# huggingface/open-muse

Hardware: AMD Instinct MI355X
Metric: images/sec/node (MaskGit train step, 256^2, bs=64/GPU) (higher is better)
Workload: dtype bf16 (transformer GEMM/attention operands; f32 accumulate, residual, norms, loss) + bf16x3 tokenizer (f32 activations, f32-class products as 3 bf16 MFMAs); parity of this mode was not measured in this run (a --full run measures it); 1 GPU; MaskGit train step: MaskGitVQGAN f16-256 encode (bf16x3) + cosine mask + MaskGitTransformer config B (configs/imagenet.yaml: hidden 768, 24 layers, 16 heads, vocab 2048, seq 257) fwd+bwd (bf16 MFMA, f32 accum/residual) + AdamW; global_batch=64, per_gpu_batch=64, resolution=256, seq_len=257, parallelism=dp1, vqgan_dtype=bf16x3, random_init=True, wgrad_stream=True

## Files before the change

include/muse_hip.h:

```cpp
#ifndef MUSE_HIP_H
#define MUSE_HIP_H
#include <stdint.h>

#ifdef __cplusplus
extern "C" {
#endif

enum { MUSE_F32 = 0, MUSE_BF16 = 1, MUSE_F16 = 2  };
enum { MUSE_ERR_BAD_ARG = -1, MUSE_ERR_ALIGN = -2, MUSE_ERR_UNSUPPORTED = -3 };

int muse_version(void);

typedef struct muse_gemm_desc {
  const void* A;
  const void* B;
  void* C;
  const void* bias;
  const void* rowvec;
  const void* residual;
  int32_t dtype;
  int32_t out_dtype;
  int32_t layout_a, layout_b;
  int32_t M, N, K;
  int32_t batch, zdiv;
  int64_t lda, ldb, ldc, ldr;
  int64_t sA0, sA1, sB0, sB1, sC0, sC1;
  float alpha;
  int32_t accumulate;
  int32_t act;
  int32_t split_k;
  int64_t split_stride;
} muse_gemm_desc;
int muse_gemm(const muse_gemm_desc* d, void* stream);
int muse_gemm_tile(const muse_gemm_desc* d);
int muse_gemm_x3(const muse_gemm_desc* d, int64_t a_lo, int64_t b_lo, void* stream);
int muse_gemm_path(const muse_gemm_desc* d);

int muse_gemm_group_ok(const muse_gemm_desc* d, int32_t n, int32_t split_k);
int muse_gemm_group(const muse_gemm_desc* d, int32_t n, int32_t split_k, void* stream);

int muse_transpose(const void* in, void* out, int32_t dtype, int32_t rows, int32_t cols, int64_t ld_in, int64_t ld_out,
                   int32_t batch, int64_t stride_in, int64_t stride_out, void* stream);

int muse_layernorm_fwd(const void* x, int32_t x_dtype, const float* w, const float* residual, void* y, int32_t y_dtype,
                       float* mean, float* rstd, int32_t rows, int32_t cols, float eps, void* stream);
int muse_layernorm_bwd(const void* dy, int32_t dy_dtype, const void* x, int32_t x_dtype, const float* w,
                       const float* mean, const float* rstd, const float* dres, void* dx, int32_t dx_dtype,
                       void* dx_bf16, float* dw_partial, int32_t nblk, int32_t rows, int32_t cols, void* stream);
int muse_layernorm_bwd_nblk(int32_t rows);
int muse_layernorm_pair_fwd(const void* ao, const float* x, const float* w_post, const float* w_pre, float* x1, void* ln2,
                            float* mean_post, float* rstd_post, float* mean_pre, float* rstd_pre, int32_t rows, int32_t cols,
                            float eps, void* stream);
int muse_layernorm_pair_bwd(const void* dln2, const float* x1, const float* w_pre, const float* mean_pre, const float* rstd_pre,
                            const float* dres, const void* ao, const float* w_post, const float* mean_post, const float* rstd_post,
                            float* dx1, void* dao, float* dw_partial_pre, float* dw_partial_post, int32_t nblk, int32_t rows,
                            int32_t cols, void* stream);
int muse_colsum(const float* in, float* out, int32_t rows, int32_t cols, int32_t accumulate, void* stream);
int muse_add_rowvec(float* x, const float* b, int64_t rows, int32_t cols, void* stream);
int muse_bias_grad_rows_per_block(void);
int muse_bias_grad_partial(const void* dy, int32_t dtype, float* partial, int64_t rows, int32_t cols, int64_t ld, void* stream);

int muse_softmax_fwd(const void* x, void* y, int32_t dtype, int64_t rows, int32_t cols, int64_t ld, void* stream);
int muse_softmax_bwd(const void* p, const void* dp, void* ds, int32_t dtype, int64_t rows, int32_t cols, int64_t ld,
                     void* stream);

typedef struct muse_attn_desc {
  const void* q;
  const void* k;
  const void* v;
  void* o;
  int64_t ldq, ldk, ldv, ldo;
  int64_t bsq, bsk, bsv, bso;
  int32_t batch, heads, head_dim, seq_q, seq_kv;
  float alpha;
} muse_attn_desc;
int muse_attention_seq_pad(int32_t seq);
int muse_attention_fwd_ex(const muse_attn_desc* d, float* lse, void* stream);
int muse_attention_bwd_ex(const muse_attn_desc* d, const void* d_o, int64_t lddo, int64_t bsdo, const float* lse, float* dsum,
                          void* dq, int64_t lddq, int64_t bsdq, void* dk, int64_t lddk, int64_t bsdk, void* dv, int64_t lddv,
                          int64_t bsdv, void* stream);
int muse_attention_x3_fwd(const muse_attn_desc* d, float* lse, void* o_planes, int64_t o_lo, int32_t half, float scale, int32_t* stats,
                          void* stream);
int muse_attention_x3_bwd(const muse_attn_desc* d, const void* d_o, int64_t lddo, int64_t bsdo, const float* lse, void* dq,
                          int64_t lddq, int64_t bsdq, void* dk, int64_t lddk, int64_t bsdk, void* dv, int64_t lddv, int64_t bsdv,
                          void* dq_planes, int64_t dq_lo, void* dk_planes, int64_t dk_lo, void* dv_planes, int64_t dv_lo, int32_t half,
                          float scale, int32_t* stats, void* stream);
int muse_attention_x3_fwd_stream(const muse_attn_desc* d, float* lse, void* o_planes, int64_t o_lo, int32_t half, float scale,
                                 int32_t* stats, void* stream);
int muse_attention_x3_bwd_stream(const muse_attn_desc* d, const float* d_o, int64_t lddo, int64_t bsdo, const float* lse, float* dsum,
// ... 211 lines not shown
```

open-muse_amd/csrc/gemm.hip:

```cpp
#include "gemm_core.h"
#include "gemm256.h"
#include "gemm_p.h"
#include "../../include/muse_hip.h"

template <typename T, typename TC, int BM>
static int dispatch_bm(const GemmParams& p, int la, int lb, int batch, hipStream_t s) {
  constexpr int NT = BM * 2;
  if (la == 0 && lb == 0) return launch_gemm<T, TC, 0, 0, BM, PlainLoader<T, 0, BM, NT>, PlainLoader<T, 0, 128, NT>>(p, batch, s);
  if (la == 0 && lb == 1) return launch_gemm<T, TC, 0, 1, BM, PlainLoader<T, 0, BM, NT>, PlainLoader<T, 1, 128, NT>>(p, batch, s);
  if (la == 1 && lb == 1) return launch_gemm<T, TC, 1, 1, BM, PlainLoader<T, 1, BM, NT>, PlainLoader<T, 1, 128, NT>>(p, batch, s);
  if (la == 1 && lb == 0) return launch_gemm<T, TC, 1, 0, BM, PlainLoader<T, 1, BM, NT>, PlainLoader<T, 0, 128, NT>>(p, batch, s);
  return MUSE_ERR_BAD_ARG;
}
template <typename T, typename TC>
static int dispatch_layout(const GemmParams& p, int la, int lb, int batch, hipStream_t s) {
  return use_bm256(p, batch) ? dispatch_bm<T, TC, 256>(p, la, lb, batch, s) : dispatch_bm<T, TC, 128>(p, la, lb, batch, s);
}

static int fill_params(const muse_gemm_desc* d, GemmParams& p) {
  if (!d || !d->A || !d->B || !d->C) return MUSE_ERR_BAD_ARG;
  const int esz = (d->dtype == MUSE_BF16 || d->dtype == MUSE_F16) ? 2 : 4;
  const int ch = 16 / esz;
  if ((d->lda % ch) || (d->ldb % ch) || (((uintptr_t)d->A) & 15) || (((uintptr_t)d->B) & 15)) return MUSE_ERR_ALIGN;
  if ((d->sA0 % ch) || (d->sA1 % ch) || (d->sB0 % ch) || (d->sB1 % ch)) return MUSE_ERR_ALIGN;
  {
    const int64_t ra = d->layout_a == 0 ? d->M : d->K, ca = d->layout_a == 0 ? d->K : d->M;
    const int64_t rb = d->layout_b == 0 ? d->N : d->K, cb = d->layout_b == 0 ? d->K : d->N;
    if (((ra - 1) * d->lda + ca + ch) * esz >= (1LL << 32) || ((rb - 1) * d->ldb + cb + ch) * esz >= (1LL << 32)) return MUSE_ERR_UNSUPPORTED;
  }
  p.A = d->A; p.B = d->B; p.C = d->C;
  p.bias = (const float*)d->bias; p.rowvec = (const float*)d->rowvec; p.residual = d->residual;
  p.M = d->M; p.N = d->N; p.K = d->K;
  p.lda = d->lda; p.ldb = d->ldb; p.ldc = d->ldc; p.ldr = d->ldr;
  p.zdiv = d->zdiv > 0 ? d->zdiv : 1;
  p.sA0 = d->sA0; p.sA1 = d->sA1; p.sB0 = d->sB0; p.sB1 = d->sB1; p.sC0 = d->sC0; p.sC1 = d->sC1;
  p.alpha = d->alpha; p.accumulate = d->accumulate; p.act = d->act;
  p.split_k = d->split_k > 1 ? d->split_k : 1;
  p.split_stride = p.split_k > 1 ? d->split_stride : 0;
  if (p.split_k > 1 && (d->out_dtype != MUSE_F32 || d->bias || d->rowvec || d->residual || d->act)) return MUSE_ERR_BAD_ARG;
  p.cH = p.cW = p.cCin = p.cKS = p.cUps = 0; p.cCinShift = -1;
  p.a_lo = p.b_lo = 0;
  return 0;
}

static bool takes_gemm256(const muse_gemm_desc* d, const GemmParams& p, int batch) {
  if (d->dtype == MUSE_F16) {
    return d->out_dtype == MUSE_F32 && d->M >= 128 && d->N >= 128 && d->K >= 64 && gemm256_ok<float>(p, d->layout_a, d->layout_b);
  }
  if (d->dtype != MUSE_BF16) return false;
  const bool pers = (d->out_dtype == MUSE_BF16 || d->out_dtype == MUSE_F32) &&
                    gemm256p_takes(p, d->layout_a, d->layout_b, batch, d->out_dtype == MUSE_F32);
  if (!gemm256_preferred(p, d->layout_a, d->layout_b, batch, pers)) return false;
  if (d->out_dtype == MUSE_BF16) return gemm256_ok<bf16_t>(p, d->layout_a, d->layout_b);
  if (d->out_dtype == MUSE_F32) return gemm256_ok<float>(p, d->layout_a, d->layout_b);
  return false;
}

extern "C" int muse_gemm_tile(const muse_gemm_desc* d) {
  GemmParams p;
  const int rc = fill_params(d, p);
  if (rc) return rc;
  if (takes_gemm256(d, p, d->batch > 0 ? d->batch : 1)) return 256;
  return d->dtype == MUSE_F16 ? MUSE_ERR_UNSUPPORTED : 128;
}

extern "C" int muse_gemm_path(const muse_gemm_desc* d) {
  GemmParams p;
  const int rc = fill_params(d, p);
  if (rc) return rc;
  const int batch = d->batch > 0 ? d->batch : 1;
  if (!takes_gemm256(d, p, batch)) return d->dtype == MUSE_F16 ? MUSE_ERR_UNSUPPORTED : 128;
  return gemm256p_takes(p, d->layout_a, d->layout_b, batch, d->out_dtype == MUSE_F32) ? 257 : 256;
}

extern "C" int muse_gemm(const muse_gemm_desc* d, void* stream) {
  GemmParams p;
  const int rc = fill_params(d, p);
  if (rc) return rc;
  const int batch = d->batch > 0 ? d->batch : 1;
  hipStream_t s = (hipStream_t)stream;
  if (d->dtype == MUSE_F16 && !takes_gemm256(d, p, batch)) return MUSE_ERR_UNSUPPORTED;
  if (takes_gemm256(d, p, batch)) {
    const bool half_ops = d->dtype == MUSE_F16;
    if (gemm256p_takes(p, d->layout_a, d->layout_b, batch, d->out_dtype == MUSE_F32)) {
      const int rp = launch_gemm256p(p, d->layout_a, d->layout_b, d->out_dtype == MUSE_F32, s, half_ops);
      if (rp != -1) return rp;
    }
    if (half_ops) return launch_gemm256_f16(p, d->layout_a, d->layout_b, batch, s);
    if (d->out_dtype == MUSE_BF16) return launch_gemm256<bf16_t>(p, d->layout_a, d->layout_b, batch, s);
    return launch_gemm256<float>(p, d->layout_a, d->layout_b, batch, s);
  }
  if (d->dtype == MUSE_BF16) {
    if (d->out_dtype == MUSE_BF16) return dispatch_layout<bf16_t, bf16_t>(p, d->layout_a, d->layout_b, batch, s);
    if (d->out_dtype == MUSE_F32) return dispatch_layout<bf16_t, float>(p, d->layout_a, d->layout_b, batch, s);
  } else if (d->dtype == MUSE_F32 && d->out_dtype == MUSE_F32) {
    return dispatch_layout<float, float>(p, d->layout_a, d->layout_b, batch, s);
  }
  return MUSE_ERR_BAD_ARG;
}

extern "C" int muse_gemm_x3(const muse_gemm_desc* d, int64_t a_lo, int64_t b_lo, void* stream) {
  GemmParams p;
  const int rc = fill_params(d, p);
  if (rc) return rc;
  if (d->dtype != MUSE_BF16 || d->out_dtype != MUSE_F32 || d->batch > 1 || d->act) return MUSE_ERR_UNSUPPORTED;
  if (a_lo <= 0 || b_lo <= 0 || (a_lo & 7) || (b_lo & 7)) return MUSE_ERR_ALIGN;
  if (d->M < 128 || d->N < 128 || d->K < 64 || !gemm256_ok<float>(p, d->layout_a, d->layout_b)) return MUSE_ERR_UNSUPPORTED;
  {
    p.a_lo = a_lo; p.b_lo = b_lo;
  }
  return launch_gemm256_x3<float>(p, d->layout_a, d->layout_b, (hipStream_t)stream);
}

static int group_fill(const muse_gemm_desc* d, int n, int split_k, g256::GroupParams& gp) {
  if (!d || n < 1 || n > g256::MAXG || split_k < 1) return MUSE_ERR_BAD_ARG;
  int start = 0;
  for (int i = 0; i < n; ++i) {
    if ((d[i].dtype != MUSE_BF16 && d[i].dtype != MUSE_F16) || d[i].dtype != d[0].dtype || d[i].out_dtype != MUSE_F32 || d[i].layout_a != 1 ||
        d[i].layout_b != 1)
      return MUSE_ERR_UNSUPPORTED;
    if ((d[i].batch > 1) || d[i].bias || d[i].rowvec || d[i].residual || d[i].act) return MUSE_ERR_UNSUPPORTED;
    muse_gemm_desc di = d[i];
    di.split_k = split_k;
    if (split_k > 1 && di.split_stride == 0) return MUSE_ERR_BAD_ARG;
    const int rc = fill_params(&di, gp.p[i]);
// ... 30 lines not shown
```

open-muse_amd/csrc/gemm256p.h:

```cpp
#pragma once
#include "gemm256.h"

namespace g256p {
using namespace g256;

constexpr int TK_OFF = LDS_BYTES;
constexpr int LDS_BYTES_P = LDS_BYTES + 64;

struct Sched {
  int ntm_full, ntn, nstrip, q, r;
  __host__ __device__ int count(int x) const {
    const int s0 = (x - r) & 7;
    return q + (x < r ? 1 : 0) + (s0 < nstrip ? (nstrip - s0 + 7) / 8 : 0);
  }
  __device__ __forceinline__ bool decode(int x, int l, int& m0, int& n0) const {
    const int full = q + (x < r ? 1 : 0);
    if (l < 0) return false;
    if (l < full) {
      const int id = (x < r ? x * (q + 1) : r * (q + 1) + (x - r) * q) + l;
      constexpr int GM = 4;
      const int grp = id / (GM * ntn), first_m = grp * GM;
      const int gm = min(ntm_full - first_m, GM), in_grp = id - grp * (GM * ntn);
      m0 = (first_m + in_grp % gm) * BM;
      n0 = (in_grp / gm) * BN;
      return true;
    }
    const int s = ((x - r) & 7) + 8 * (l - full);
    if (s < nstrip) { m0 = ntm_full * BM; n0 = s * BN; return true; }
    return false;
  }
};

struct PArgs {
  GemmParams g;
  Sched sched;
  unsigned* counters;
  int nk2;
  int dyn;
  int epi;
  int staux;
  int stagger;
};

template <int L>
struct DmaP {
  rsrc_t rs;
  unsigned voff0[4];
  unsigned kk0, oob, kstep, ld2;
  unsigned vmask;
  unsigned r0off;
  int kend, R, rel0;
  __device__ __forceinline__ void init(const bf16_t* ptr, long ld, int R_, int K, int wave, int lane) {
    kend = K; R = R_;
    const long cols = L == 0 ? K : R_, rows = L == 0 ? R_ : K;
    const unsigned bytes = (unsigned)(((rows - 1) * ld + (cols + 7) / 8 * 8) * 2);
    rs = make_rsrc(ptr, bytes);
    oob = (bytes + 15u) & ~15u;
    ld2 = (unsigned)(ld * 2);
    vmask = 0; r0off = 0;
    if constexpr (L == 0) {
      const int r8 = lane >> 3, pc = lane & 7;
      kstep = 128u;
      kk0 = (unsigned)((pc ^ (r8 >> 1)) * 8);
      rel0 = wave * 32 + r8;
#pragma unroll
      for (int j = 0; j < 4; ++j) {
        const int row = (wave * 4 + j) * 8 + r8;
        const int csrc = pc ^ ((row >> 1) & 7);
        voff0[j] = (unsigned)(((long)row * ld + csrc * 8) * 2);
      }
    } else {
      const int half = lane >> 5, pos = lane & 31;
      kstep = (unsigned)(64 * ld * 2);
      kk0 = (unsigned)(wave * 8 + half);
      rel0 = 0;
#pragma unroll
      for (int j = 0; j < 4; ++j) {
        const int kr = wave * 8 + j * 2 + half;
        const int csrc = pos ^ (km_sw(kr) << 1);
        voff0[j] = (unsigned)(((long)kr * ld + csrc * 8) * 2);
      }
    }
  }
  __device__ __forceinline__ int rel(int j, int wave, int lane) const {
    if constexpr (L == 0) return rel0 + 8 * j;
    const int half = lane >> 5, pos = lane & 31, kr = wave * 8 + j * 2 + half;
    return (pos ^ (km_sw(kr) << 1)) * 8;
  }
  __device__ __forceinline__ void set_tile(int r0, bool valid, int wave, int lane) {
    unsigned m = 0;
#pragma unroll
    for (int j = 0; j < 4; ++j) m |= (valid && (r0 + rel(j, wave, lane)) < R) ? (1u << j) : 0u;
    vmask = m;
    r0off = L == 0 ? (unsigned)r0 * ld2 : (unsigned)r0 * 2u;
  }
  __device__ __forceinline__ unsigned kk(int j) const { return L == 0 ? (kk0 ^ ((unsigned)(j & 1) << 5)) : (kk0 + 2u * j); }
  template <int LDS_OFF, int J>
  __device__ __forceinline__ void issue1(unsigned char* smem, int kt, int wave) const {
    const bool ok = ((unsigned)kt * 64u + kk(J)) < (unsigned)kend && ((vmask >> J) & 1u);
    const unsigned vo = ok ? voff0[J] : oob;
    __builtin_amdgcn_raw_ptr_buffer_load_lds(rs, (lds_void_t*)(smem + LDS_OFF + (wave * 4 + J) * 1024), 16, (int)vo,
                                             (int)((unsigned)kt * kstep + r0off), 0, 0);
  }
  template <int LDS_OFF>
  __device__ __forceinline__ void issue(unsigned char* smem, int kt, int wave) const {
    issue1<LDS_OFF, 0>(smem, kt, wave); issue1<LDS_OFF, 1>(smem, kt, wave);
    issue1<LDS_OFF, 2>(smem, kt, wave); issue1<LDS_OFF, 3>(smem, kt, wave);
  }
};

enum { M_NORMAL = 0, M_FIRST = 1, M_LAST = 2, M_PUBLISH = 3 };

template <typename TC, int AL, int BL, bool H = false>
struct PipeP {
  static constexpr bool F32OUT = sizeof(TC) == 4;
  static constexpr int RA = AL ? 2 : 1, RB = BL ? 2 : 1, NB = NI * RB;
  static constexpr int NSLOT = 4, DIST = NSLOT - 1;
  static constexpr int GB1 = 8 - DIST, GBAR = 16 - DIST;
  static constexpr int NST = F32OUT ? 32 : 16;
  DmaP<AL> da;
  DmaP<BL> db;
  Frags<AL, MI> fa;
  Frags<BL, NI> fb;
  f32x4 acc[MI][NI];
  bf16x8 ring[NSLOT];
  bf16x8 bk[2][NI];
  unsigned char* smem;
  Sched sched;
  unsigned* counters;
  int nk2, dyn, epi, staux, stagger, M, N;
  unsigned ldc;
  float alpha;
// ... 136 lines not shown
  }

  __device__ __forceinline__ void epilogue(int m0, int n0) {
    if (alpha != 1.f) {
#pragma unroll
      for (int i = 0; i < MI; ++i)
#pragma unroll
        for (int j = 0; j < NI; ++j) acc[i][j] *= alpha;
    }
    if (epi == 3) {
#pragma unroll
      for (int i = 0; i < MI; ++i)
        asm volatile("" ::"v"(acc[i][0]), "v"(acc[i][1]), "v"(acc[i][2]), "v"(acc[i][3]));
      return;
    }
    int ln = lane;
    asm volatile("" : "+v"(ln));
    const int pr = ln & 15, g = ln >> 4;
    const int rowlim = M - m0 - wr - pr;
    constexpr unsigned E = (unsigned)sizeof(TC);
    const unsigned soff = (unsigned)m0 * ldc * E + (unsigned)n0 * E, rstep = 16u * ldc * E;
    const unsigned rowb = (unsigned)(wr + pr) * ldc * E;
    if constexpr (F32OUT) {
      const int cb = wc + 4 * g;
      unsigned vb[NI];
#pragma unroll
      for (int j = 0; j < NI; ++j) vb[j] = (n0 + cb + 16 * j) < N ? rowb + (unsigned)(cb + 16 * j) * 4u : oobC;
#pragma unroll
      for (int i = 0; i < MI; ++i) {
        const bool rowok = 16 * i < rowlim;
#pragma unroll
        for (int j = 0; j < NI; ++j)
          __builtin_amdgcn_raw_buffer_store_b128(__builtin_bit_cast(u32x4, acc[i][j]), rsC, (int)(rowok ? vb[j] : oobC),
                                                 (int)(soff + (unsigned)i * rstep), 0);
        __builtin_amdgcn_sched_barrier(0);
      }
    } else {
      if (epi == 0) {
        const int cb = wc + 4 * g;
        unsigned vb[NI];
#pragma unroll
        for (int j = 0; j < NI; ++j) vb[j] = (n0 + cb + 16 * j) < N ? rowb + (unsigned)(cb + 16 * j) * 2u : oobC;
#pragma unroll
        for (int i = 0; i < MI; ++i) {
          const bool rowok = 16 * i < rowlim;
#pragma unroll
          for (int j = 0; j < NI; ++j) {
            const u32x2 w = {pack2_bf16(acc[i][j][0], acc[i][j][1]), pack2_bf16(acc[i][j][2], acc[i][j][3])};
            __builtin_amdgcn_raw_buffer_store_b64(w, rsC, (int)(rowok ? vb[j] : oobC), (int)(soff + (unsigned)i * rstep), 0);
          }
          __builtin_amdgcn_sched_barrier(0);
        }
      } else {
        const int cg = 16 * (g & 1) + 8 * (g >> 1);
        if (epi == 1) {
          unsigned vb[2];
#pragma unroll
          for (int q = 0; q < 2; ++q) vb[q] = (n0 + wc + cg + 32 * q) < N ? rowb + (unsigned)(wc + cg + 32 * q) * 2u : oobC;
#pragma unroll
          for (int i = 0; i < MI; ++i) {
            const bool rowok = 16 * i < rowlim;
#pragma unroll
            for (int q = 0; q < 2; ++q) {
              u32x4 w;
              swapped_chunk(i, q, w);
              store16(w, rowok ? vb[q] : oobC, soff + (unsigned)i * rstep);
            }
            __builtin_amdgcn_sched_barrier(0);
          }
        } else {
          const int odd = pr & 1;
          const int col = wc + cg + 32 * odd;
          const int rl0 = rowlim + odd;
          const unsigned vb0 = (n0 + col) < N ? rowb - (unsigned)odd * ldc * 2u + (unsigned)col * 2u : oobC;
          const unsigned vb1 = (n0 + col) < N ? vb0 + ldc * 2u : oobC;
#pragma unroll
          for (int i = 0; i < MI; ++i) {
            u32x4 c0, c1, d0, d1;
            swapped_chunk(i, 0, c0);
            swapped_chunk(i, 1, c1);
#pragma unroll
            for (int e = 0; e < 4; ++e) {
              const unsigned from1 = (unsigned)__builtin_amdgcn_update_dpp(0, (int)c1[e], 0xB1, 0xf, 0xf, false);
              const unsigned from0 = (unsigned)__builtin_amdgcn_update_dpp(0, (int)c0[e], 0xB1, 0xf, 0xf, false);
              d0[e] = odd ? from1 : c0[e];
              d1[e] = odd ? c1[e] : from0;
            }
            store16(d0, 16 * i < rl0 ? vb0 : oobC, soff + (unsigned)i * rstep);
            store16(d1, 16 * i + 1 < rl0 ? vb1 : oobC, soff + (unsigned)i * rstep);
            __builtin_amdgcn_sched_barrier(0);
          }
        }
      }
    }
  }

  __device__ __forceinline__ void tiles(int& m0, int& n0) {
    for (;;) {
      ktile<0, M_FIRST>();
      ktile<1, M_PUBLISH>();
      for (int it = 2; it < nk2 - 2; it += 2) {
        ktile<0, M_NORMAL>();
        ktile<1, M_NORMAL>();
      }
      ktile<0, M_LAST>();
      ktile<1, M_NORMAL>();
      issue_piece<1, 3>(1); issue_piece<1, 4>(1); issue_piece<1, 5>(1); issue_piece<1, 6>(1); issue_piece<1, 7>(1);
      fence();
      epilogue(m0, n0);
      fence();
      if (!has_next) return;
      m0 = nm0; n0 = nn0;
      const bool ld = init_acc(m0, n0);
      fence();
      pend = !ld && epi != 3;
    }
  }

  __device__ __forceinline__ void run(int m0, int n0) {
    if (dyn && stagger > 1) {
      const long wait = (long)((blockIdx.x >> 3) % stagger) * ((long)nk2 * 2500L / stagger);
      const long t0 = (long)__builtin_amdgcn_s_memtime();
      while ((long)__builtin_amdgcn_s_memtime() - t0 < wait) __builtin_amdgcn_s_sleep(16);
    }
    da.set_tile(m0, true, wave, lane);
    db.set_tile(n0, true, wave, lane);
    da.template issue<A_BASE>(smem, 0, wave);
    db.template issue<B_BASE>(smem, 0, wave);
    da.template issue<A_BASE + TILE>(smem, 1, wave);
    db.template issue<B_BASE + TILE>(smem, 1, wave);
    fence();
    const bool loads = init_acc(m0, n0);
    fence();
    if (loads) asm volatile("s_waitcnt vmcnt(40)" ::: "memory");
    else asm volatile("s_waitcnt vmcnt(8)" ::: "memory");
    __builtin_amdgcn_s_barrier();
    __builtin_amdgcn_sched_barrier(0);
    fb.template read_range<0, 0, 0, NI>(bk[0]);
    prologue_a<0>();
    __builtin_amdgcn_sched_barrier(0);
    kti = 0;
    pend = false;
    has_next = false;
    tiles(m0, n0);
    asm volatile("s_waitcnt vmcnt(0) lgkmcnt(0)" ::: "memory");
  }
};

template <typename TC, int AL, int BL, bool H = false>
__global__ __launch_bounds__(512, 2) void kernel(PArgs a) {
  extern __shared__ __attribute__((aligned(16))) unsigned char smem[];
  const GemmParams& p = a.g;
  const int lane = threadIdx.x & 63, wave = __builtin_amdgcn_readfirstlane(threadIdx.x >> 6);
  const int xcd = blockIdx.x & 7, nbx = gridDim.x >> 3;

  int m0, n0;
  if (a.sched.decode(xcd, blockIdx.x >> 3, m0, n0)) {
    PipeP<TC, AL, BL, H> pp;
    pp.smem = smem; pp.sched = a.sched; pp.counters = a.counters; pp.nk2 = a.nk2; pp.dyn = a.dyn; pp.epi = a.epi; pp.staux = a.staux; pp.stagger = a.stagger;
    pp.M = p.M; pp.N = p.N; pp.ldc = (unsigned)p.ldc; pp.alpha = p.alpha;
    pp.wave = wave; pp.lane = lane; pp.xcd = xcd; pp.nbx = nbx;
    pp.wr = (wave >> 2) * 128; pp.wc = (wave & 3) * 64;
    pp.tk = 0;
    pp.da.init((const bf16_t*)p.A, p.lda, p.M, p.K, wave, lane);
    pp.db.init((const bf16_t*)p.B, p.ldb, p.N, p.K, wave, lane);
    pp.fa.init(A_BASE, pp.wr, lane);
    pp.fb.init(B_BASE, pp.wc, lane);
    {
      const unsigned bytes = (unsigned)(((long)(p.M - 1) * p.ldc + p.N) * (long)sizeof(TC));
      pp.rsC = make_rsrc(p.C, bytes);
      pp.oobC = (bytes + 15u) & ~15u;
    }
    pp.init_src = nullptr; pp.ldI = 0; pp.oobI = 0; pp.rsI = pp.rsC;
    if constexpr (sizeof(TC) == 4) {
      if (p.residual || p.accumulate) {
        pp.init_src = p.residual ? p.residual : (const void*)p.C;
        pp.ldI = (unsigned)(p.residual ? p.ldr : p.ldc);
        const unsigned bytes = (unsigned)(((long)(p.M - 1) * pp.ldI + p.N) * 4L);
        pp.rsI = make_rsrc(pp.init_src, bytes);
        pp.oobI = (bytes + 15u) & ~15u;
      }
    }
    pp.run(m0, n0);
  }
  if (a.dyn && threadIdx.x == 0) {
    const unsigned left = __hip_atomic_fetch_add(a.counters + 8, 1u, __ATOMIC_RELAXED, __HIP_MEMORY_SCOPE_AGENT);
    if (left == gridDim.x - 1) {
#pragma unroll
      for (int x = 0; x < 9; ++x) __hip_atomic_exchange(a.counters + x, 0u, __ATOMIC_RELAXED, __HIP_MEMORY_SCOPE_AGENT);
    }
  }
}

}
```

open-muse_amd/csrc/gemm_p.h:

```cpp
#pragma once
#include "gemm_core.h"
bool gemm256p_takes(const GemmParams& p, int la, int lb, int batch, bool f32_out);
int launch_gemm256p(const GemmParams& p, int la, int lb, bool f32_out, hipStream_t stream, bool half_ops = false);
```

open-muse_amd/csrc/gemm_p.hip:

```cpp
#include "gemm256p.h"
#include "gemm_p.h"
#include <mutex>
#include <stdio.h>

namespace {

constexpr int kMaxDev = 16;
struct Slots {
  unsigned* base = nullptr;
  hipStream_t streams[64];
  int n = 0;
  int cus = 0;
  bool failed = false;
};
std::mutex g_mu;
Slots g_slots[kMaxDev];

Slots* slots_of_current_device() {
  int dev = 0;
  if (hipGetDevice(&dev) != hipSuccess || dev < 0 || dev >= kMaxDev) { (void)hipGetLastError(); return nullptr; }
  Slots& S = g_slots[dev];
  if (S.failed) return nullptr;
  if (!S.base) {
    hipDeviceProp_t prop;
    if (hipGetDeviceProperties(&prop, dev) != hipSuccess || hipMalloc((void**)&S.base, 64 * 64) != hipSuccess ||
        hipMemset(S.base, 0, 64 * 64) != hipSuccess) {
      (void)hipGetLastError();
      S.failed = true;
      S.base = nullptr;
      return nullptr;
    }
    S.cus = prop.multiProcessorCount;
  }
  return &S;
}

unsigned* counters_for(hipStream_t s, int* cus) {
  std::lock_guard<std::mutex> lk(g_mu);
  hipStreamCaptureStatus cap = hipStreamCaptureStatusNone;
  if (hipStreamIsCapturing(s, &cap) != hipSuccess) (void)hipGetLastError();
  if (cap != hipStreamCaptureStatusNone) return nullptr;
  Slots* S = slots_of_current_device();
  if (!S) return nullptr;
  *cus = S->cus;
  for (int i = 0; i < S->n; ++i)
    if (S->streams[i] == s) return S->base + i * 16;
  if (S->n == 64) return nullptr;
  S->streams[S->n] = s;
  return S->base + (S->n++) * 16;
}

#define P_REJECT(why) do { if (getenv("MUSE_G256P_DEBUG")) fprintf(stderr, "[g256p] %dx%dx%d la%d lb%d out%d: %s\n", p.M, p.N, p.K, la, lb, (int)sizeof(TC), why); return false; } while (0)
template <typename TC>
bool eligible(const GemmParams& p, int la, int lb, int batch) {
  constexpr long E = (long)sizeof(TC);
  if (batch != 1 || p.split_k > 1 || p.act != 0 || p.bias || p.rowvec) P_REJECT("batch / split-K / activation / bias / row vector");
  if (la != 0 || (sizeof(TC) == 4 && lb != 0)) P_REJECT("operand layout");
  if (p.K <= 128) P_REJECT("K <= 128");
  if (sizeof(TC) == 2 && (p.residual || p.accumulate)) P_REJECT("bf16 residual / accumulate");
  if (sizeof(TC) == 4 && ((p.residual && p.accumulate) || ((p.residual || p.accumulate) && p.alpha != 1.f))) P_REJECT("residual + accumulate / alpha");
  if (!gemm256_ok<TC>(p, la, lb)) P_REJECT("gemm256_ok");
  const long ra = la == 0 ? p.M : p.K, rb = lb == 0 ? p.N : p.K;
  if ((ra * p.lda + 16) * 2 >= (1L << 31) || (rb * p.ldb + 16) * 2 >= (1L << 31)) P_REJECT("operand >= 2 GiB");
  if (((long)p.M * p.ldc + 16) * E >= (1L << 31)) P_REJECT("C >= 2 GiB");
  if (p.residual && ((long)p.M * p.ldr + 16) * E >= (1L << 31)) P_REJECT("residual >= 2 GiB");
  return true;
}

template <typename TC, int AL, int BL, bool H = false>
int launch(const GemmParams& p, hipStream_t stream) {
  int cus = 0;
  unsigned* counters = counters_for(stream, &cus);
  if (!counters || cus < 8) {
    if (getenv("MUSE_G256P_DEBUG")) fprintf(stderr, "[g256p] no queue slot (counters %p, %d CUs)\n", (void*)counters, cus);
    return -1;
  }
  g256p::PArgs a;
  a.g = p;
  a.counters = counters;
  g256p::Sched& sc = a.sched;
  sc.ntm_full = p.M / 256;
  sc.ntn = (p.N + 255) / 256;
  sc.nstrip = (p.M % 256) ? sc.ntn : 0;
  const int nfull = sc.ntm_full * sc.ntn;
  sc.q = nfull / 8; sc.r = nfull % 8;
  int longest = 0;
  for (int x = 0; x < 8; ++x) longest = sc.count(x) > longest ? sc.count(x) : longest;
  const int per_xcd = cus / 8;
  const int nbx = longest < per_xcd ? longest : per_xcd;
  a.dyn = longest > nbx;
  a.nk2 = (((p.K + 63) / 64) + 1) & ~1;
  static const int epi = []() { const char* e = getenv("MUSE_G256P_EPI"); return e ? atoi(e) : 2; }();
  a.epi = epi;
  static const int staux = []() { const char* e = getenv("MUSE_G256P_STAUX"); return e ? atoi(e) : 0; }();
  static const int stagger = []() { const char* e = getenv("MUSE_G256P_STAGGER"); return e ? atoi(e) : 1; }();
  a.staux = staux;
  a.stagger = stagger;
  auto kern = g256p::kernel<TC, AL, BL, H>;
  set_max_dynamic_lds((const void*)kern, g256p::LDS_BYTES_P);
  hipLaunchKernelGGL(kern, dim3(8 * nbx), dim3(512), g256p::LDS_BYTES_P, stream, a);
  return (int)hipGetLastError();
}

int launch_l(const GemmParams& p, int la, int lb, bool f32_out, hipStream_t s, bool half_ops) {
  if (la != 0) return -1;
  if (half_ops) return (f32_out && lb == 0) ? launch<float, 0, 0, true>(p, s) : -1;
  if (f32_out) return lb == 0 ? launch<float, 0, 0>(p, s) : -1;
  return lb == 0 ? launch<bf16_t, 0, 0>(p, s) : launch<bf16_t, 0, 1>(p, s);
}

}

bool gemm256p_takes(const GemmParams& p, int la, int lb, int batch, bool f32_out) {
  const char* e = getenv("MUSE_G256P");
  if (e && e[0] == '0') return false;
  return f32_out ? eligible<float>(p, la, lb, batch) : eligible<bf16_t>(p, la, lb, batch);
}

int launch_gemm256p(const GemmParams& p, int la, int lb, bool f32_out, hipStream_t stream, bool half_ops) {
  return launch_l(p, la, lb, f32_out, stream, half_ops);
}
```

open-muse_amd/muse/_hip.py:

```python
from __future__ import annotations

import ctypes as C
import os

import torch

F32, BF16, F16 = 0, 1, 2
_HERE = os.path.dirname(os.path.abspath(__file__))
LIB_PATH = os.environ.get("MUSE_HIP_LIB") or os.path.join(_HERE, "libmuse_hip.so")
_lib = None

c_void_p, c_int, c_i64, c_float = C.c_void_p, C.c_int32, C.c_int64, C.c_float


class GemmDesc(C.Structure):
    _fields_ = [
        ("A", c_void_p), ("B", c_void_p), ("C", c_void_p),
        ("bias", c_void_p), ("rowvec", c_void_p), ("residual", c_void_p),
        ("dtype", c_int), ("out_dtype", c_int), ("layout_a", c_int), ("layout_b", c_int),
        ("M", c_int), ("N", c_int), ("K", c_int), ("batch", c_int), ("zdiv", c_int),
        ("lda", c_i64), ("ldb", c_i64), ("ldc", c_i64), ("ldr", c_i64),
        ("sA0", c_i64), ("sA1", c_i64), ("sB0", c_i64), ("sB1", c_i64), ("sC0", c_i64), ("sC1", c_i64),
        ("alpha", c_float), ("accumulate", c_int), ("act", c_int), ("split_k", c_int), ("split_stride", c_i64),
    ]


class AttnDesc(C.Structure):
    _fields_ = [
        ("q", c_void_p), ("k", c_void_p), ("v", c_void_p), ("o", c_void_p),
        ("ldq", c_i64), ("ldk", c_i64), ("ldv", c_i64), ("ldo", c_i64),
        ("bsq", c_i64), ("bsk", c_i64), ("bsv", c_i64), ("bso", c_i64),
        ("batch", c_int), ("heads", c_int), ("head_dim", c_int), ("seq_q", c_int), ("seq_kv", c_int),
        ("alpha", c_float),
    ]


_IMG = (c_int, c_float, c_void_p)

SIGNATURES = {
    "muse_version": [],
    "muse_gemm": [C.POINTER(GemmDesc), c_void_p],
    "muse_gemm_x3": [C.POINTER(GemmDesc), c_i64, c_i64, c_void_p],
    "muse_gemm_tile": [C.POINTER(GemmDesc)],
    "muse_gemm_path": [C.POINTER(GemmDesc)],
    "muse_transpose": [c_void_p, c_void_p, c_int, c_int, c_int, c_i64, c_i64, c_int, c_i64, c_i64, c_void_p],
    "muse_layernorm_fwd": [c_void_p, c_int, c_void_p, c_void_p, c_void_p, c_int, c_void_p, c_void_p, c_int, c_int,
                           c_float, c_void_p],
    "muse_layernorm_bwd": [c_void_p, c_int, c_void_p, c_int, c_void_p, c_void_p, c_void_p, c_void_p, c_void_p, c_int,
                           c_void_p, c_void_p, c_int, c_int, c_int, c_void_p],
    "muse_layernorm_bwd_nblk": [c_int],
    "muse_layernorm_pair_fwd": [c_void_p] * 10 + [c_int, c_int, c_float, c_void_p],
    "muse_layernorm_pair_bwd": [c_void_p] * 14 + [c_int, c_int, c_int, c_void_p],
    "muse_colsum": [c_void_p, c_void_p, c_int, c_int, c_int, c_void_p],
    "muse_add_rowvec": [c_void_p, c_void_p, c_i64, c_int, c_void_p],
    "muse_bias_grad_rows_per_block": [],
    "muse_bias_grad_partial": [c_void_p, c_int, c_void_p, c_i64, c_int, c_i64, c_void_p],
    "muse_softmax_fwd": [c_void_p, c_void_p, c_int, c_i64, c_int, c_i64, c_void_p],
    "muse_softmax_bwd": [c_void_p, c_void_p, c_void_p, c_int, c_i64, c_int, c_i64, c_void_p],
    "muse_attention_seq_pad": [c_int],
    "muse_attention_fwd_ex": [C.POINTER(AttnDesc), c_void_p, c_void_p],
    "muse_attention_bwd_ex": [C.POINTER(AttnDesc), c_void_p, c_i64, c_i64, c_void_p, c_void_p, c_void_p, c_i64, c_i64, c_void_p,
                              c_i64, c_i64, c_void_p, c_i64, c_i64, c_void_p],
    "muse_attention_x3_fwd": [C.POINTER(AttnDesc), c_void_p, c_void_p, c_i64, *_IMG, c_void_p],
    "muse_attention_x3_bwd": [C.POINTER(AttnDesc), c_void_p, c_i64, c_i64, c_void_p, c_void_p, c_i64, c_i64, c_void_p, c_i64, c_i64, c_void_p,
                              c_i64, c_i64, c_void_p, c_i64, c_void_p, c_i64, c_void_p, c_i64, *_IMG, c_void_p],
    "muse_attention_x3_fwd_stream": [C.POINTER(AttnDesc), c_void_p, c_void_p, c_i64, *_IMG, c_void_p],
    "muse_attention_x3_bwd_stream": [C.POINTER(AttnDesc), c_void_p, c_i64, c_i64, c_void_p, c_void_p, c_void_p, c_i64, c_i64, c_void_p, c_i64, c_i64,
                                     c_void_p, c_i64, c_i64, c_void_p, c_i64, c_void_p, c_i64, c_void_p, c_i64, *_IMG, c_void_p],
    "muse_attention_x3_merge": [c_void_p, c_i64, c_void_p, c_i64, c_int, c_void_p, c_void_p, c_void_p, c_i64, c_int, c_int, c_int, *_IMG,
                                c_void_p],
    "muse_sum_parts_strided": [c_void_p, c_i64, c_int, c_i64, c_int, c_void_p, c_i64, c_int, c_void_p],
    "muse_attention_fwd": [c_void_p, c_void_p, c_void_p, c_int, c_int, c_int, c_int, c_float, c_void_p],
    "muse_attention_bwd": [c_void_p, c_void_p, c_void_p, c_void_p, c_void_p, c_void_p, c_int, c_int, c_int, c_int, c_float,
                           c_void_p],
    "muse_glu_fwd": [c_void_p, c_void_p, c_int, c_i64, c_int, c_void_p],
    "muse_glu_bwd": [c_void_p, c_void_p, c_void_p, c_int, c_i64, c_int, c_void_p],
    "muse_glu_fwd_x3": [c_void_p, c_void_p, c_void_p, c_i64, c_int, *_IMG, c_void_p],
    "muse_glu_bwd_x3": [c_void_p, c_void_p, c_void_p, c_void_p, c_i64, c_int, *_IMG, c_void_p],
    "muse_ffn_mid_rows_per_block": [],
    "muse_ffn_mid_fwd": [c_void_p, c_void_p, c_void_p, c_void_p, c_void_p, c_void_p, c_int, c_int, c_int, c_float, c_void_p],
    "muse_ffn_mid_bwd": [c_void_p, c_void_p, c_void_p, c_void_p, c_void_p, c_void_p, c_void_p, c_void_p, c_int, c_int, c_int,
                         c_void_p],
    "muse_gelu_fwd": [c_void_p, c_void_p, c_int, c_i64, c_void_p],
    "muse_gelu_bwd": [c_void_p, c_void_p, c_void_p, c_int, c_i64, c_void_p],
    "muse_gelu_bwd_f32_bf16": [c_void_p, c_void_p, c_void_p, c_i64, c_void_p],
    "muse_embed_fwd": [c_void_p, c_void_p, c_void_p, c_void_p, c_int, c_int, c_int, c_int, c_void_p],
    "muse_embed_bwd": [c_void_p, c_void_p, c_void_p, c_void_p, c_void_p, c_int, c_int, c_int, c_int, c_int, c_void_p],
    "muse_embed_bwd_scratch_floats": [c_int, c_int],
    "muse_embed_bwd2": [c_void_p, c_void_p, c_void_p, c_void_p, c_void_p, c_i64, c_int, c_int, c_int, c_int, c_int, c_void_p],
    "muse_embed_bwd2_scratch_bytes": [c_int, c_int, c_int, c_int],
    "muse_cross_entropy_fwd": [c_void_p, c_int, c_void_p, c_void_p, c_void_p, c_void_p, c_i64, c_int, c_i64, c_float,
                               c_void_p],
    "muse_cross_entropy_bwd": [c_void_p, c_int, c_void_p, c_void_p, c_void_p, c_void_p, c_void_p, c_int, c_i64, c_int,
                               c_i64, c_float, c_void_p],
    "muse_soft_ce_fwd": [c_void_p, c_void_p, c_void_p, c_void_p, c_void_p, c_void_p, c_void_p, c_i64, c_int, c_int, c_i64, c_void_p],
    "muse_soft_ce_bwd": [c_void_p, c_void_p, c_void_p, c_void_p, c_void_p, c_void_p, c_void_p, c_void_p, c_int, c_i64, c_int, c_int,
                         c_i64, c_i64, c_void_p],
# ... 141 lines not shown
```

open-muse_amd/muse/ops.py:

```python
from __future__ import annotations

import ctypes as C
import math
import os
import weakref

import torch

from . import _hip
from ._hip import BF16, F16, F32, GemmDesc, check, dt, lib, ptr, require_gpu, stream

USE_TR = os.environ.get("MUSE_GEMM_TR", "1") != "0"


def _esz(t):
    return t.element_size()


_PROF = None


PROF_BYTES = {}


# ... 229 lines not shown
    def __enter__(self):
        self.prev = (_F32_AS_F16[0], _F16_IMAGES[0])
        _F32_AS_F16[0] = self.on
        if self.on:
            _F16_IMAGES[0] = self.images
        return self

    def __exit__(self, *exc):
        _F32_AS_F16[0], _F16_IMAGES[0] = self.prev
        if self.on and self.images is not None and self.images.backward:
            _F16_GUARDS.add(self.images)
        return False


def _image_args(gradient, *planes):
    half = _F32_AS_F16[0]
    for p in planes:
        if p is not None and p.dtype != (torch.float16 if half else torch.bfloat16):
            raise _hip.MuseHipError(f"operand image of dtype {p.dtype} in a{'n f16' if half else ' bf16x3'} pass")
    if not half:
        return 0, 1.0, None
    im = _F16_IMAGES[0]
    return 1, im.grad_scale if gradient else 1.0, im._ensure_stats().data_ptr()


def cast_to_f16(t, scale=1.0, stats=None):
    require_gpu(t)
    if t.dtype != torch.float32 or not t.is_contiguous():
        raise _hip.MuseHipError("cast_to_f16: contiguous f32 tensor")
    out = torch.empty(t.shape, dtype=torch.float16, device=t.device)
    check(lib().muse_cast_f32_to_f16(t.data_ptr(), out.data_ptr(), t.numel(), float(scale), ptr(stats), stream()), "muse_cast_f32_to_f16")
    out._muse_scale = float(scale)
    return out


def _f16_operands_ok(A, B, M, N, K, la, lb, lda, ldb):
    return (A.dim() == 2 and B.dim() == 2 and A.is_contiguous() and B.is_contiguous() and K % 8 == 0 and lda % 8 == 0 and ldb % 8 == 0
            and A.stride(0) == lda and B.stride(0) == ldb and A.shape[1 if la == 0 else 0] == K and B.shape[1 if lb == 0 else 0] == K
            and A.shape[0 if la == 0 else 1] >= M and B.shape[0 if lb == 0 else 1] >= N and M >= 128 and N >= 128 and K >= 64
            and A.numel() * 2 < (1 << 31) and B.numel() * 2 < (1 << 31))


def _f16_kernel_takes(A, B, c_ptr, M, N, K, la, lb, lda, ldb, ldc, residual=None, ldr=0):
    d = GemmDesc()
    d.A, d.B, d.C = A.data_ptr(), B.data_ptr(), c_ptr
    d.dtype, d.out_dtype, d.layout_a, d.layout_b = F16, F32, la, lb
    d.M, d.N, d.K, d.batch, d.zdiv = M, N, K, 1, 1
    d.lda, d.ldb, d.ldc, d.ldr = lda, ldb, ldc, ldr
    d.residual = ptr(residual)
    d.alpha = 1.0
    return lib().muse_gemm_tile(C.byref(d)) == 256


def _gemm_f16(A, B, C_, M, N, K, la, lb, lda, ldb, ldc, c_off, alpha, bias, rowvec, residual, ldr, accumulate, a_off, b_off):
    if a_off or b_off or not _f16_operands_ok(A, B, M, N, K, la, lb, lda, ldb):
        return False
    if not _f16_kernel_takes(A, B, C_.data_ptr() + c_off * 4, M, N, K, la, lb, lda, ldb, ldc, residual, ldr):
        return False
    im = _F16_IMAGES[0]
    a16 = im.image(A, im.grad_scale if im.backward else 1.0)
    b16 = im.image(B, 1.0)
    gemm(a16, b16, C_, M, N, K, la=la, lb=lb, lda=lda, ldb=ldb, ldc=ldc, c_off=c_off, alpha=alpha, bias=bias, rowvec=rowvec,
         residual=residual, ldr=ldr, accumulate=accumulate)
    return True


def f16_wgrad_operands(dy, x, M=None, lda=None):
    if not (_F32_AS_F16[0] and dy.dtype == torch.float32 and x.dtype == torch.float32 and dy.dim() == 2 and x.dim() == 2
            and (lda is None or lda == dy.stride(0)) and dy.shape[0] == x.shape[0]):
        return None
    N = M if M is not None else dy.shape[1]
    if not (_f16_operands_ok(dy, x, N, x.shape[1], dy.shape[0], 1, 1, dy.stride(0), x.stride(0))
            and _f16_kernel_takes(dy, x, dy.data_ptr(), N, x.shape[1], dy.shape[0], 1, 1, dy.stride(0), x.stride(0), x.shape[1])):
        return None
    im = _F16_IMAGES[0]
    return im.image(dy, im.grad_scale), im.image(x, 1.0)


_F32_AS_BF16X3 = [False]
_X3_IMAGES = [None]


class X3Images:

    def __init__(self, recent=12):
        self.persist, self.lru, self.recent, self.backward = {}, {}, int(recent), False
        self.hits = self.misses = self.produced = 0

    def clear(self):
        self.persist.clear()
        self.lru.clear()

    @staticmethod
    def _key(t, layout, lo_pos):
        return (t.data_ptr(), tuple(t.shape), tuple(t.stride()), t._version, layout, lo_pos)

    def get(self, t, layout, K, lo_pos, last_use=False):
        key = self._key(t, layout, lo_pos)
        hit = self.persist.pop(key, None) if last_use else self.persist.get(key)
        if hit is not None and last_use:
            self._recent(key, hit)
        if hit is None:
            hit = self.lru.get(key)
        if hit is not None:
            self.hits += 1
            return hit[1], hit[2]
# ... 1737 lines not shown
```

Measured before the change: 1254 images/s.

## Add column-mapped bf16 epilogue to persistent GEMM with permuted B loading

Adds epilogue modes 8/9 for the persistent 256 GEMM with bf16 output and N a multiple of 256. In these modes the B rows are loaded in a permuted order (cm_row) with a matching LDS swizzle and fragment addresses, so accumulators pack directly into contiguous output chunks without the swapped_chunk shuffle. Mode 9 becomes the default, and env reads are no longer cached statically. It also exposes a query function reporting which epilogue a GEMM would use. This risks correctness if the permutation and swizzle do not match, and adds a getenv call on every launch.

```diff
diff --git a/include/muse_hip.h b/include/muse_hip.h
--- a/include/muse_hip.h
+++ b/include/muse_hip.h
@@ -35,6 +35,7 @@
 int muse_gemm_tile(const muse_gemm_desc* d);
 int muse_gemm_x3(const muse_gemm_desc* d, int64_t a_lo, int64_t b_lo, void* stream);
 int muse_gemm_path(const muse_gemm_desc* d);
+int muse_gemm_epilogue(const muse_gemm_desc* d);
 
 int muse_gemm_group_ok(const muse_gemm_desc* d, int32_t n, int32_t split_k);
 int muse_gemm_group(const muse_gemm_desc* d, int32_t n, int32_t split_k, void* stream);
diff --git a/open-muse_amd/csrc/gemm.hip b/open-muse_amd/csrc/gemm.hip
--- a/open-muse_amd/csrc/gemm.hip
+++ b/open-muse_amd/csrc/gemm.hip
@@ -71,6 +71,15 @@
   const int batch = d->batch > 0 ? d->batch : 1;
   if (!takes_gemm256(d, p, batch)) return d->dtype == MUSE_F16 ? MUSE_ERR_UNSUPPORTED : 128;
   return gemm256p_takes(p, d->layout_a, d->layout_b, batch, d->out_dtype == MUSE_F32) ? 257 : 256;
+}
+
+extern "C" int muse_gemm_epilogue(const muse_gemm_desc* d) {
+  const int path = muse_gemm_path(d);
+  if (path < 0) return path;
+  if (path != 257) return 0;
+  GemmParams p;
+  fill_params(d, p);
+  return gemm256p_epilogue(p, d->out_dtype == MUSE_F32);
 }
 
 extern "C" int muse_gemm(const muse_gemm_desc* d, void* stream) {
diff --git a/open-muse_amd/csrc/gemm256p.h b/open-muse_amd/csrc/gemm256p.h
--- a/open-muse_amd/csrc/gemm256p.h
+++ b/open-muse_amd/csrc/gemm256p.h
@@ -6,6 +6,9 @@
 
 constexpr int TK_OFF = LDS_BYTES;
 constexpr int LDS_BYTES_P = LDS_BYTES + 64;
+
+__host__ __device__ constexpr int cm_row(int row) { return (row & ~0x1c) | ((row & 0xc) << 1) | ((row & 0x10) >> 2); }
+__host__ __device__ constexpr int km_sw_cm(int kr) { return (kr & 1) | (((kr >> 1) & 1) << 2) | (((kr >> 3) & 1) << 3); }
 
 struct Sched {
   int ntm_full, ntn, nstrip, q, r;
@@ -50,7 +53,7 @@
   unsigned vmask;
   unsigned r0off;
   int kend, R, rel0;
-  __device__ __forceinline__ void init(const bf16_t* ptr, long ld, int R_, int K, int wave, int lane) {
+  __device__ __forceinline__ void init(const bf16_t* ptr, long ld, int R_, int K, int wave, int lane, bool cmap = false) {
     kend = K; R = R_;
     const long cols = L == 0 ? K : R_, rows = L == 0 ? R_ : K;
     const unsigned bytes = (unsigned)(((rows - 1) * ld + (cols + 7) / 8 * 8) * 2);
@@ -67,7 +70,7 @@
       for (int j = 0; j < 4; ++j) {
         const int row = (wave * 4 + j) * 8 + r8;
         const int csrc = pc ^ ((row >> 1) & 7);
-        voff0[j] = (unsigned)(((long)row * ld + csrc * 8) * 2);
+        voff0[j] = (unsigned)(((long)(cmap ? cm_row(row) : row) * ld + csrc * 8) * 2);
       }
     } else {
       const int half = lane >> 5, pos = lane & 31;
@@ -77,7 +80,7 @@
 #pragma unroll
       for (int j = 0; j < 4; ++j) {
         const int kr = wave * 8 + j * 2 + half;
-        const int csrc = pos ^ (km_sw(kr) << 1);
+        const int csrc = pos ^ (cmap ? km_sw_cm(kr) : (km_sw(kr) << 1));
         voff0[j] = (unsigned)(((long)kr * ld + csrc * 8) * 2);
       }
     }
@@ -320,46 +323,67 @@
           __builtin_amdgcn_sched_barrier(0);
         }
       } else {
-        const int cg = 16 * (g & 1) + 8 * (g >> 1);
-        if (epi == 1) {
-          unsigned vb[2];
-#pragma unroll
-          for (int q = 0; q < 2; ++q) vb[q] = (n0 + wc + cg + 32 * q) < N ? rowb + (unsigned)(wc + cg + 32 * q) * 2u : oobC;
-#pragma unroll
-          for (int i = 0; i < MI; ++i) {
-            const bool rowok = 16 * i < rowlim;
-#pragma unroll
-            for (int q = 0; q < 2; ++q) {
-              u32x4 w;
-              swapped_chunk(i, q, w);
-              store16(w, rowok ? vb[q] : oobC, soff + (unsigned)i * rstep);
-            }
-            __builtin_amdgcn_sched_barrier(0);
-          }
-        } else {
-          const int odd = pr & 1;
-          const int col = wc + cg + 32 * odd;
-          const int rl0 = rowlim + odd;
-          const unsigned vb0 = (n0 + col) < N ? rowb - (unsigned)odd * ldc * 2u + (unsigned)col * 2u : oobC;
-          const unsigned vb1 = (n0 + col) < N ? vb0 + ldc * 2u : oobC;
-#pragma unroll
-          for (int i = 0; i < MI; ++i) {
-            u32x4 c0, c1, d0, d1;
-            swapped_chunk(i, 0, c0);
-            swapped_chunk(i, 1, c1);
-#pragma unroll
-            for (int e = 0; e < 4; ++e) {
-              const unsigned from1 = (unsigned)__builtin_amdgcn_update_dpp(0, (int)c1[e], 0xB1, 0xf, 0xf, false);
-              const unsigned from0 = (unsigned)__builtin_amdgcn_update_dpp(0, (int)c0[e], 0xB1, 0xf, 0xf, false);
-              d0[e] = odd ? from1 : c0[e];
-              d1[e] = odd ? c1[e] : from0;
-            }
-            store16(d0, 16 * i < rl0 ? vb0 : oobC, soff + (unsigned)i * rstep);
-            store16(d1, 16 * i + 1 < rl0 ? vb1 : oobC, soff + (unsigned)i * rstep);
-            __builtin_amdgcn_sched_barrier(0);
-          }
-        }
-      }
+        if (epi == 1) store_segments<false>(16 * (g & 1) + 8 * (g >> 1), pr, g, n0, rowb, rowlim, soff, rstep);
+        else if (epi == 8) store_segments<true>(8 * g, pr, g, n0, rowb, rowlim, soff, rstep);
+        else if (epi == 9) store_lines<true>(8 * g, pr, g, n0, rowb, rowlim, soff, rstep);
+        else store_lines<false>(16 * (g & 1) + 8 * (g >> 1), pr, g, n0, rowb, rowlim, soff, rstep);
+      }
+    }
+  }
+  template <bool CM>
+  __device__ __forceinline__ void chunk(int i, int q, int g, u32x4& w) {
+    if constexpr (!CM) {
+      swapped_chunk(i, q, w);
+    } else {
+      const unsigned x0 = pack2_bf16(acc[i][2 * q][0], acc[i][2 * q][1]), x1 = pack2_bf16(acc[i][2 * q][2], acc[i][2 * q][3]);
+      const unsigned y0 = pack2_bf16(acc[i][2 * q + 1][0], acc[i][2 * q + 1][1]), y1 = pack2_bf16(acc[i][2 * q + 1][2], acc[i][2 * q + 1][3]);
+      if constexpr (BL == 1) {
+        const bool flip = g & 1;
+        w = u32x4{flip ? y0 : x0, flip ? y1 : x1, flip ? x0 : y0, flip ? x1 : y1};
+      } else {
+        w = u32x4{x0, x1, y0, y1};
+      }
+    }
+  }
+  template <bool CM>
+  __device__ __forceinline__ void store_segments(int cg, int pr, int g, int n0, unsigned rowb, int rowlim, unsigned soff, unsigned rstep) {
+    unsigned vb[2];
+#pragma unroll
+    for (int q = 0; q < 2; ++q) vb[q] = (n0 + wc + cg + 32 * q) < N ? rowb + (unsigned)(wc + cg + 32 * q) * 2u : oobC;
+#pragma unroll
+    for (int i = 0; i < MI; ++i) {
+      const bool rowok = 16 * i < rowlim;
+#pragma unroll
+      for (int q = 0; q < 2; ++q) {
+        u32x4 w;
+        chunk<CM>(i, q, g, w);
+        store16(w, rowok ? vb[q] : oobC, soff + (unsigned)i * rstep);
+      }
+      __builtin_amdgcn_sched_barrier(0);
+    }
+  }
+  template <bool CM>
+  __device__ __forceinline__ void store_lines(int cg, int pr, int g, int n0, unsigned rowb, int rowlim, unsigned soff, unsigned rstep) {
+    const int odd = pr & 1;
+    const int col = wc + cg + 32 * odd;
+    const int rl0 = rowlim + odd;
+    const unsigned vb0 = (n0 + col) < N ? rowb - (unsigned)odd * ldc * 2u + (unsigned)col * 2u : oobC;
+    const unsigned vb1 = (n0 + col) < N ? vb0 + ldc * 2u : oobC;
+#pragma unroll
+    for (int i = 0; i < MI; ++i) {
+      u32x4 c0, c1, d0, d1;
+      chunk<CM>(i, 0, g, c0);
+      chunk<CM>(i, 1, g, c1);
+#pragma unroll
+      for (int e = 0; e < 4; ++e) {
+        const unsigned from1 = (unsigned)__builtin_amdgcn_update_dpp(0, (int)c1[e], 0xB1, 0xf, 0xf, false);
+        const unsigned from0 = (unsigned)__builtin_amdgcn_update_dpp(0, (int)c0[e], 0xB1, 0xf, 0xf, false);
+        d0[e] = odd ? from1 : c0[e];
+        d1[e] = odd ? c1[e] : from0;
+      }
+      store16(d0, 16 * i < rl0 ? vb0 : oobC, soff + (unsigned)i * rstep);
+      store16(d1, 16 * i + 1 < rl0 ? vb1 : oobC, soff + (unsigned)i * rstep);
+      __builtin_amdgcn_sched_barrier(0);
     }
   }
 
@@ -430,10 +454,21 @@
     pp.wave = wave; pp.lane = lane; pp.xcd = xcd; pp.nbx = nbx;
     pp.wr = (wave >> 2) * 128; pp.wc = (wave & 3) * 64;
     pp.tk = 0;
+    const bool cmap = sizeof(TC) == 2 && (a.epi == 8 || a.epi == 9);
     pp.da.init((const bf16_t*)p.A, p.lda, p.M, p.K, wave, lane);
-    pp.db.init((const bf16_t*)p.B, p.ldb, p.N, p.K, wave, lane);
+    pp.db.init((const bf16_t*)p.B, p.ldb, p.N, p.K, wave, lane, cmap);
     pp.fa.init(A_BASE, pp.wr, lane);
     pp.fb.init(B_BASE, pp.wc, lane);
+    if constexpr (BL == 1 && sizeof(TC) == 2) {
+      if (cmap) {
+        const int pl = lane & 15, kr = 8 * (lane >> 4) + (pl >> 2), cc = pl & 3;
+#pragma unroll
+        for (int f = 0; f < NI; ++f) {
+          const int ch = (pp.wc >> 3) + 4 * (f >> 1) + cc;
+          pp.fb.addr[f] = (unsigned)(B_BASE + kr * 512 + ((ch ^ km_sw_cm(kr)) << 4) + ((cc ^ f) & 1) * 8);
+        }
+      }
+    }
     {
       const unsigned bytes = (unsigned)(((long)(p.M - 1) * p.ldc + p.N) * (long)sizeof(TC));
       pp.rsC = make_rsrc(p.C, bytes);
diff --git a/open-muse_amd/csrc/gemm_p.h b/open-muse_amd/csrc/gemm_p.h
--- a/open-muse_amd/csrc/gemm_p.h
+++ b/open-muse_amd/csrc/gemm_p.h
@@ -1,4 +1,5 @@
 #pragma once
 #include "gemm_core.h"
 bool gemm256p_takes(const GemmParams& p, int la, int lb, int batch, bool f32_out);
+int gemm256p_epilogue(const GemmParams& p, bool f32_out);
 int launch_gemm256p(const GemmParams& p, int la, int lb, bool f32_out, hipStream_t stream, bool half_ops = false);
diff --git a/open-muse_amd/csrc/gemm_p.hip b/open-muse_amd/csrc/gemm_p.hip
--- a/open-muse_amd/csrc/gemm_p.hip
+++ b/open-muse_amd/csrc/gemm_p.hip
@@ -67,6 +67,14 @@
   return true;
 }
 
+template <typename TC>
+int epilogue_mode(const GemmParams& p) {
+  const char* e = getenv("MUSE_G256P_EPI");
+  const int epi = e ? atoi(e) : 9;
+  if (epi >= 4) return ((epi == 8 || epi == 9) && sizeof(TC) == 2 && p.N % 256 == 0) ? epi : 2;
+  return epi;
+}
+
 template <typename TC, int AL, int BL, bool H = false>
 int launch(const GemmParams& p, hipStream_t stream) {
   int cus = 0;
@@ -90,12 +98,11 @@
   const int nbx = longest < per_xcd ? longest : per_xcd;
   a.dyn = longest > nbx;
   a.nk2 = (((p.K + 63) / 64) + 1) & ~1;
-  static const int epi = []() { const char* e = getenv("MUSE_G256P_EPI"); return e ? atoi(e) : 2; }();
-  a.epi = epi;
-  static const int staux = []() { const char* e = getenv("MUSE_G256P_STAUX"); return e ? atoi(e) : 0; }();
-  static const int stagger = []() { const char* e = getenv("MUSE_G256P_STAGGER"); return e ? atoi(e) : 1; }();
-  a.staux = staux;
-  a.stagger = stagger;
+  a.epi = epilogue_mode<TC>(p);
+  const char* e_staux = getenv("MUSE_G256P_STAUX");
+  const char* e_stagger = getenv("MUSE_G256P_STAGGER");
+  a.staux = e_staux ? atoi(e_staux) : 0;
+  a.stagger = e_stagger ? atoi(e_stagger) : 1;
   auto kern = g256p::kernel<TC, AL, BL, H>;
   set_max_dynamic_lds((const void*)kern, g256p::LDS_BYTES_P);
   hipLaunchKernelGGL(kern, dim3(8 * nbx), dim3(512), g256p::LDS_BYTES_P, stream, a);
@@ -117,6 +124,8 @@
   return f32_out ? eligible<float>(p, la, lb, batch) : eligible<bf16_t>(p, la, lb, batch);
 }
 
+int gemm256p_epilogue(const GemmParams& p, bool f32_out) { return f32_out ? epilogue_mode<float>(p) : epilogue_mode<bf16_t>(p); }
+
 int launch_gemm256p(const GemmParams& p, int la, int lb, bool f32_out, hipStream_t stream, bool half_ops) {
   return launch_l(p, la, lb, f32_out, stream, half_ops);
 }
diff --git a/open-muse_amd/muse/_hip.py b/open-muse_amd/muse/_hip.py
--- a/open-muse_amd/muse/_hip.py
+++ b/open-muse_amd/muse/_hip.py
@@ -43,6 +43,7 @@
     "muse_gemm_x3": [C.POINTER(GemmDesc), c_i64, c_i64, c_void_p],
     "muse_gemm_tile": [C.POINTER(GemmDesc)],
     "muse_gemm_path": [C.POINTER(GemmDesc)],
+    "muse_gemm_epilogue": [C.POINTER(GemmDesc)],
     "muse_transpose": [c_void_p, c_void_p, c_int, c_int, c_int, c_i64, c_i64, c_int, c_i64, c_i64, c_void_p],
     "muse_layernorm_fwd": [c_void_p, c_int, c_void_p, c_void_p, c_void_p, c_int, c_void_p, c_void_p, c_int, c_int,
                            c_float, c_void_p],
diff --git a/open-muse_amd/muse/ops.py b/open-muse_amd/muse/ops.py
--- a/open-muse_amd/muse/ops.py
+++ b/open-muse_amd/muse/ops.py
@@ -305,6 +305,19 @@
     return lib().muse_gemm_tile(C.byref(d)) == 256
 
 
+def gemm_epilogue(A, B, C_, M, N, K, *, la=0, lb=0, lda, ldb, ldc):
+    d = GemmDesc()
+    d.A, d.B, d.C = A.data_ptr(), B.data_ptr(), C_.data_ptr()
+    d.dtype, d.out_dtype, d.layout_a, d.layout_b = BF16, (F32 if C_.dtype == torch.float32 else BF16), la, lb
+    d.M, d.N, d.K, d.batch, d.zdiv = M, N, K, 1, 1
+    d.lda, d.ldb, d.ldc = lda, ldb, ldc
+    d.alpha = 1.0
+    epi = lib().muse_gemm_epilogue(C.byref(d))
+    if epi < 0:
+        check(epi, "muse_gemm_epilogue")
+    return epi
+
+
 def _gemm_f16(A, B, C_, M, N, K, la, lb, lda, ldb, ldc, c_off, alpha, bias, rowvec, residual, ldr, accumulate, a_off, b_off):
     if a_off or b_off or not _f16_operands_ok(A, B, M, N, K, la, lb, lda, ldb):
         return False
```

New measurement: 1253 images/s. About the same (-0.0%).
